# DearCaat/MHIM-MIL

Hardware: AMD Instinct MI355X
Metric: patch-instances/sec through MHIM fwd+bwd, N=10k D=1024 (higher is better)
Workload: dtype f32; 1 GPU; c2: MHIM(ABMIL) train step, one bag N=10000 D=1024 per GPU per step (teacher fwd + select + student fwd + bwd + Adam + EMA); rotating_bags_per_gpu=8, matrix_core_form=bf16x3, parallelism=dp1, launch=hipGraph replay, one graph per resident bag

## Files before the change

include/mhimx.h:

```cpp
#ifndef MHIMX_H
#define MHIMX_H

#include <stdint.h>

#ifdef __cplusplus
extern "C" {
#endif

#define MHIMX_VERSION 620

enum { MHIMX_ACT_NONE = 0, MHIMX_ACT_RELU = 1, MHIMX_ACT_GELU = 2, MHIMX_ACT_TANH = 3 };

enum { MHIMX_PREC_F32 = 0, MHIMX_PREC_F16S = 1, MHIMX_PREC_BF16X3 = 2 };

const char* mhimx_last_error(void);
int mhimx_version(void);


typedef struct {
  const float* A; int64_t lda; const int64_t* rows;
  const float* B; int64_t ldb;
  float* C; int64_t ldc;
  int64_t M, N, K;
  const float* bias;
// ... 282 lines not shown
                          float* colsum_out, int32_t accumulate, void* ws, int64_t ws_bytes, mhimx_reduce_list* defer );
int mhimx_rows_dpre_image_c(void* stream, const float* dH_compact, const void* dact16, const int64_t* rows, int64_t L, int64_t E, void* img,
                            float* colsum_out, int32_t accumulate, void* ws, int64_t ws_bytes, mhimx_reduce_list* defer );
int mhimx_rows_dpre_image_k(void* stream, const float* dH, const void* dact16, const uint8_t* keep, int64_t N, int64_t E, void* img,
                            float* colsum_out, int32_t accumulate, void* ws, int64_t ws_bytes, mhimx_reduce_list* defer );
typedef struct {
  const void* img;
  const float* X; int64_t ldx; int64_t n_bag_rows;
  const int64_t* rows;
  int64_t L, E, D;
  float* C; int64_t ldc; int32_t accumulate;
  float* ws; int64_t ws_floats;
  mhimx_reduce_list* defer;
  int32_t ride_tail;
  const void* ximg;
} mhimx_bag_wgrad_args;
int64_t mhimx_wgrad_ws_floats(int64_t L, int64_t E, int64_t D);
int mhimx_bag_wgrad(void* stream, const mhimx_bag_wgrad_args* a);
int64_t mhimx_wgrad_multi_ws_floats(int64_t L, int64_t E, int64_t D, int32_t n_bags);
int mhimx_bag_wgrad_multi(void* stream, const mhimx_bag_wgrad_args* bags, int32_t n_bags);
int mhimx_shard_flags(void* stream, const int64_t* rows_all, int64_t R, int64_t Lk, int64_t lo, int64_t n, int64_t k_tokens,
                      int32_t tokens_live, uint8_t* excl);
int mhimx_shard_gather(void* stream, const float* H, int64_t E, const int64_t* rows, int64_t R, int64_t lo, int64_t n, float* out);
int mhimx_shard_scatter(void* stream, const float* dX, int64_t E, const int64_t* rows, int64_t R, int64_t lo, int64_t n, float* dH);
int mhimx_colsum(void* stream, const float* X, int64_t M, int64_t E, float* out, int32_t accumulate,
                 void* ws, int64_t ws_bytes);

int mhimx_head_fwd_bwd(void* stream, const float* z, const float* t, const float* wp, const float* bp,
                       const int64_t* label_dev, int64_t E, int64_t C, float temp_t, float main_alpha,
                       float aux_alpha, float inv_accum, float* logits, float* losses, float* g_z, float* d_wp,
                       float* d_bp, int32_t accumulate, const float* g_logits_in, const float* g_cl_in);

int mhimx_softmax_cols(void* stream, const float* x, float* y, int64_t M, int64_t C, float alpha);
// ... 45 lines not shown
  int32_t act, da_act;
  int32_t attn2score;
  float drop_p_teacher, drop_p_student;
  float merge_drop_p, merge_mm;
  float temp_t, main_alpha, aux_alpha;
  mhimx_step_params student, teacher;
  mhimx_step_grads grad;
  float* p; float* g; float* m; float* v; float* p_teacher;
  int64_t n_train, n_all;
  float lr, beta1, beta2, eps, weight_decay, ema_mm;
  const float* mm_table; int64_t mm_len; const float* lr_table; int64_t lr_len;
  uint64_t* tick; uint64_t* opt_step;
  float* q_out;
  int32_t time_project;
  void* side_stream;
} mhimx_step_cfg;
typedef struct { int64_t k_top, n_sel, len_keep, Lk, R; } mhimx_step_counts;
int mhimx_step_counts_of(int64_t N, double mask_ratio_h, double mask_ratio_hr, double merge_ratio, mhimx_step_counts* out);
typedef struct { uint64_t drop_teacher, drop_student, select, mca; } mhimx_step_seeds;
typedef struct {
  int64_t total;
  int64_t logits, losses;
  int64_t score;
  int64_t rows_all;
  int64_t H_teacher, H_student;
  int64_t dact;
  int64_t z_teacher, z_student, g_z;
  int64_t dH;
} mhimx_step_layout;
int mhimx_step_layout_of(const mhimx_step_cfg* cfg, int64_t N, const mhimx_step_counts* cnt, mhimx_step_layout* out);
// ... 284 lines not shown
```

mhim_mil_amd/_lib.py:

```python
from __future__ import annotations

import ctypes as C
import os

HERE = os.path.dirname(os.path.abspath(__file__))
LIB_PATH = os.path.join(HERE, os.environ.get("MHIMX_LIB_NAME", "libmhimx.so"))

c_f32p = C.c_void_p
c_i64p = C.c_void_p
c_u8p = C.c_void_p

ABI_VERSION = 620

ACT = {None: 0, "none": 0, "identity": 0, "relu": 1, "gelu": 2, "tanh": 3}
PREC = {"f32": 0, "f16s": 1, "bf16x3": 2}


def act_code(name, allowed):
    n = name.lower() if isinstance(name, str) else None
    return ACT[n] if n in allowed else 0


class GemmNT(C.Structure):
    _fields_ = [("A", c_f32p), ("lda", C.c_int64), ("rows", c_i64p),
# ... 15 lines not shown


class ProjScore(C.Structure):
    _fields_ = [("wa16", c_f32p), ("wc", c_f32p), ("act", C.c_int32), ("C", C.c_int32), ("s", c_f32p), ("cproj", c_f32p),
                ("pm", c_f32p), ("pl", c_f32p), ("pz", c_f32p), ("xch", c_f32p), ("gate", C.c_void_p)]


class BagProject(C.Structure):
    _fields_ = [("X", c_f32p), ("ldx", C.c_int64), ("N", C.c_int64), ("D", C.c_int64), ("E", C.c_int64),
                ("act", C.c_int32), ("n_heads", C.c_int32), ("head", ProjHead * 2), ("drop_tick", C.c_void_p), ("score0", C.c_void_p)]


class BagWgrad(C.Structure):
    _fields_ = [("img", C.c_void_p), ("X", c_f32p), ("ldx", C.c_int64), ("n_bag_rows", C.c_int64), ("rows", C.c_void_p),
                ("L", C.c_int64), ("E", C.c_int64), ("D", C.c_int64), ("C", c_f32p), ("ldc", C.c_int64), ("accumulate", C.c_int32),
                ("ws", c_f32p), ("ws_floats", C.c_int64), ("defer", C.c_void_p), ("ride_tail", C.c_int32), ("ximg", C.c_void_p)]


class PpegBand(C.Structure):
    _fields_ = [("H", C.c_int64), ("cell0", C.c_int64), ("ncell", C.c_int64), ("out0", C.c_int64), ("out1", C.c_int64)]


class PrepJob(C.Structure):
    _fields_ = [("kind", C.c_int32), ("inp", C.c_void_p), ("out", C.c_void_p), ("R", C.c_int64), ("C", C.c_int64)]


class ReduceJob(C.Structure):
    _fields_ = [("kind", C.c_int32), ("accumulate", C.c_int32), ("parts", c_f32p), ("out", c_f32p),
                ("G", C.c_int64), ("W", C.c_int64), ("ld", C.c_int64), ("K1", C.c_int64), ("K2", C.c_int64), ("ldo", C.c_int64)]


# ... 100 lines not shown

class StepGrads(C.Structure):
    _fields_ = [(n, C.c_void_p) for n in ("w1", "b1", "wa", "wc", "wp", "bp", "ln_w", "ln_b", "wkv", "wq", "wo", "bo")]


class StepCfg(C.Structure):
    _fields_ = [("D", C.c_int64), ("E", C.c_int64), ("A", C.c_int64), ("C", C.c_int64), ("k", C.c_int64),
                ("act", C.c_int32), ("da_act", C.c_int32), ("attn2score", C.c_int32),
                ("drop_p_teacher", C.c_float), ("drop_p_student", C.c_float), ("merge_drop_p", C.c_float), ("merge_mm", C.c_float),
                ("temp_t", C.c_float), ("main_alpha", C.c_float), ("aux_alpha", C.c_float),
                ("student", StepParams), ("teacher", StepParams), ("grad", StepGrads),
                ("p", C.c_void_p), ("g", C.c_void_p), ("m", C.c_void_p), ("v", C.c_void_p), ("p_teacher", C.c_void_p),
                ("n_train", C.c_int64), ("n_all", C.c_int64),
                ("lr", C.c_float), ("beta1", C.c_float), ("beta2", C.c_float), ("eps", C.c_float), ("weight_decay", C.c_float), ("ema_mm", C.c_float),
                ("mm_table", C.c_void_p), ("mm_len", C.c_int64), ("lr_table", C.c_void_p), ("lr_len", C.c_int64),
                ("tick", C.c_void_p), ("opt_step", C.c_void_p), ("q_out", C.c_void_p), ("time_project", C.c_int32), ("side_stream", C.c_void_p)]


class StepCounts(C.Structure):
    _fields_ = [("k_top", C.c_int64), ("n_sel", C.c_int64), ("len_keep", C.c_int64), ("Lk", C.c_int64), ("R", C.c_int64)]


class StepSeeds(C.Structure):
    _fields_ = [("drop_teacher", C.c_uint64), ("drop_student", C.c_uint64), ("select", C.c_uint64), ("mca", C.c_uint64)]


class StepLayout(C.Structure):
    _fields_ = [(n, C.c_int64) for n in ("total", "logits", "losses", "score", "rows_all", "H_teacher", "H_student", "dact", "z_teacher",
                                        "z_student", "g_z", "dH")]


# ... 190 lines not shown
    "mhimx_dsmil_head": (C.c_int, [_P, _P, _P, _P, _P, _P, _I64, _I64, _F, _F, _F, _F, _P, _P, _P, _P, _P]),
    "mhimx_mul_colsum": (C.c_int, [_P, _P, _P, _I64, _I64, _P, _I32, _P, _I64, _P]),
    "mhimx_rows_dpre": (C.c_int, [_P, _P, _P, _P, _I64, _I64, _P, _P, _I32, _P, _I64, _P]),
    "mhimx_bmm_affine": (C.c_int, [_P, _I32, _P, _I32, _I64, _I64, _I64, C.c_float, C.c_float]),
    "mhimx_bmm_affine2": (C.c_int, [_P, _I32, _P, _I32, _I64, _I64, _I64, C.c_float, C.c_float, _P, C.c_float, C.c_float]),
    "mhimx_bmm_affine_pair": (C.c_int, [_P, _I32, C.POINTER(GemmNT), _F, _F, _I32, C.POINTER(GemmNT), _F, _F, _I32, _I64]),
    "mhimx_shard_flags": (C.c_int, [_P, _P, _I64, _I64, _I64, _I64, _I64, _I32, _P]),
    "mhimx_shard_gather": (C.c_int, [_P, _P, _I64, _P, _I64, _I64, _I64, _P]),
    "mhimx_shard_scatter": (C.c_int, [_P, _P, _I64, _P, _I64, _I64, _I64, _P]),
    "mhimx_rows_dpre_image": (C.c_int, [_P, _P, _P, _P, _I64, _I64, _P, _P, _I32, _P, _I64, _P]),
    "mhimx_rows_dpre_image_c": (C.c_int, [_P, _P, _P, _P, _I64, _I64, _P, _P, _I32, _P, _I64, _P]),
    "mhimx_rows_dpre_image_k": (C.c_int, [_P, _P, _P, _P, _I64, _I64, _P, _P, _I32, _P, _I64, _P]),
    "mhimx_wgrad_image_bytes": (_I64, [_I64, _I64]),
    "mhimx_wgrad_ws_floats": (_I64, [_I64, _I64, _I64]),
    "mhimx_bag_wgrad": (C.c_int, [_P, _P]),
    "mhimx_bag_wgrad_multi": (C.c_int, [_P, _P, _I32]),
    "mhimx_wgrad_multi_ws_floats": (C.c_int64, [_I64, _I64, _I64, _I32]),
    "mhimx_reduce_flush": (C.c_int, [_P, _P]),
    "mhimx_cls_metrics_ws_bytes": (C.c_int64, [_I64, _I64, _I64]),
    "mhimx_cls_metrics": (C.c_int, [_P, _P, _I64, _P, _I64, _I64, _I32, _P, _I64, _P, _P, _I64]),
    "mhimx_surv_nll": (C.c_int, [_P, _P, _I64, _P, _P, _I64, _I64, _F, _F, _F, _P, _P, _P]),
    "mhimx_cindex_ws_bytes": (C.c_int64, [_I64, _I64]),
    "mhimx_cindex": (C.c_int, [_P, _P, _P, _P, _I64, _P, _I64, _F, _P, _P, _I64]),
    "mhimx_colsum": (C.c_int, [_P, _P, _I64, _I64, _P, _I32, _P, _I64]),
    "mhimx_head_fwd_bwd": (C.c_int, [_P, _P, _P, _P, _P, _P, _I64, _I64, _F, _F, _F, _F, _P, _P, _P, _P, _P, _I32, _P, _P]),
    "mhimx_head_surv_fwd_bwd": (C.c_int, [_P, _P, _P, _P, _P, _P, _P, _I64, _I64, _F, _F, _F, _F, _F, _F, _P, _P, _P, _P, _P, _P, _I32]),
    "mhimx_adam_ema": (C.c_int, [_P, _P, _P, _P, _P, _P, _I64, _I64, _I64, _F, _F, _F, _F, _F, _F, _F, _I32, _P, _P, _I64]),
    "mhimx_bmm_chain": (C.c_int, [_P, C.POINTER(BmmStep), _I32, _I32, _P]),
    "mhimx_optim_step": (C.c_int, [_P, C.POINTER(OptimArgs)]),
    "mhimx_stream_copy": (C.c_int, [_P, _P, _P, _I64]),
# ... 110 lines not shown
```

mhim_mil_amd/csrc/step.hip:

```cpp
#include <math.h>
#include <string.h>

#include "infer_tab.hpp"
#include "step_mid.hpp"

namespace mhimx {

int64_t merge2_rows_tiles(int64_t R);

namespace {

struct DagEvents {
  hipEvent_t e[64][6];
  bool have[64] = {};
  int get(hipEvent_t** out) {
    int dev = 0;
    MHIMX_HIP(hipGetDevice(&dev));
    MHIMX_CHECK_ARG(dev >= 0 && dev < 64, "step: device index %d", dev);
    if (!have[dev]) {
      for (int i = 0; i < 6; ++i) MHIMX_HIP(hipEventCreateWithFlags(&e[dev][i], hipEventDisableTiming));
      have[dev] = true;
    }
    *out = e[dev];
    return 0;
// ... 389 lines not shown
  mhimx_reduce_list lst;
  memset(&lst, 0, sizeof(lst));
  const MidImg pimg = {cv.at<char>(b.img), dact, cv.at<float>(b.ws_b)};
  if (int r = mid_bwd_rows(stream, im, fwd, bag, c.grad, 0, fuse_img ? &pimg : nullptr, dag, &lst)) return r;
  mhimx_reduce_list lst_main;
  memset(&lst_main, 0, sizeof(lst_main));
  mhimx_reduce_list* lm = dag ? &lst_main : &lst;
  if (fuse_img) {
    if (int r = dpre_merge_rows(stream, dH, dact, rows_all, R, E, cv.at<char>(b.img), b.P0, c.grad.b1, cv.at<float>(b.ws_b), b.ws_b_bytes, lm)) return r;
  } else if (int r = mhimx_rows_dpre_image(stream, dH, dact, rows_all, len_keep, E, cv.at<char>(b.img), c.grad.b1, 0, cv.at<char>(b.ws_b), b.ws_b_bytes, lm))
    return r;
  {
    mhimx_bag_wgrad_args g = {};
    g.img = cv.at<char>(b.img); g.X = X; g.ldx = ldx; g.n_bag_rows = N; g.rows = fuse_img ? cv.at<int64_t>(b.rows_img) : rows_all; g.L = b.L_img; g.E = E; g.D = D;
    g.C = c.grad.w1; g.ldc = D;
    g.accumulate = 0; g.ws = cv.at<float>(b.wg_ws); g.ws_floats = b.wg_ws_floats; g.defer = lm; g.ride_tail = update ? 1 : 0;
    if (int r = mhimx_bag_wgrad(stream, &g)) return r;
  }
  if (dag)
    if (int r = dag_edge(dag->ev[4], dag->side_st, dag->main_st)) return r;
  if (!update) return mhimx_reduce_flush(stream, lm);

  mhimx_optim_args o = optim_args_of(c, host_step, true);
  o.fold = lm;
  return mhimx_optim_step(stream, &o);
}

namespace mhimx {
namespace {

struct QChainW { float wq; float w[MHIMX_WINDOW_MAX]; };
// ... 346 lines not shown

  mhimx_reduce_list lst;
  memset(&lst, 0, sizeof(lst));
  {
    mhimx_scorer sc_b = sc;
    sc_b.wa_frag = nullptr;
    mhimx_pool_grad pg = {};
    pg.g_z = g_z; pg.dT1 = dH; pg.d_wa = c.grad.wa; pg.d_wc = c.grad.wc; pg.wa_t = wa_t; pg.accumulate = 0; pg.splits = 8; pg.defer = &lst; pg.wa_t_frag = wa_t_frag;
    if (int r = mhimx_abmil_pool_bwd(stream, &sc_b, &io, &pg)) return r;
  }
  if (int r = mhimx_rows_dpre_image(stream, dH, dact, nullptr, N, E, cv.at<char>(b.img), c.grad.b1, 0, cv.at<char>(b.ws_b), b.ws_b_bytes, &lst)) return r;
  {
    mhimx_bag_wgrad_args g = {};
    g.img = cv.at<char>(b.img); g.X = X; g.ldx = ldx; g.n_bag_rows = N; g.rows = nullptr; g.L = N; g.E = E; g.D = D;
    g.C = c.grad.w1; g.ldc = D;
    g.accumulate = 0; g.ws = cv.at<float>(b.wg_ws); g.ws_floats = b.wg_ws_floats; g.defer = &lst; g.ride_tail = update ? 1 : 0;
    if (int r = mhimx_bag_wgrad(stream, &g)) return r;
  }
  if (!update) return mhimx_reduce_flush(stream, &lst);

  mhimx_optim_args o = optim_args_of(c, host_step, false);
  o.fold = &lst;
  return mhimx_optim_step(stream, &o);
}

extern "C" int mhimx_pure_step_run_many(void* stream, const mhimx_step_cfg* cfg, int32_t n_bags, const float* const* X, const int64_t* ldx, const int64_t* N,
                                        const int64_t* const* labels_dev, const uint64_t* drop_seeds, int64_t host_step0, void* ws, int64_t ws_bytes) {
  MHIMX_CHECK_ARG(n_bags >= 1 && X && ldx && N && labels_dev && drop_seeds, "pure_step_run_many: null arguments");
  for (int32_t i = 0; i < n_bags; ++i)
    if (int r = mhimx_pure_step_run(stream, cfg, X[i], ldx[i], N[i], labels_dev[i], drop_seeds[i], host_step0 + i, ws, ws_bytes, 1)) return r;
  return 0;
// ... 2 lines not shown
```

mhim_mil_amd/csrc/wgrad.hip:

```cpp
#include <string.h>

#include "mma_tile.hpp"
#include "mca2_side.hpp"
#include "reduce_jobs.hpp"

namespace mhimx {

constexpr int WBI = 128, WBN = 256, WBK = 32, WTHREADS = 512;
constexpr int WA_BYTES = WBI * 128, WB_BYTES = WBN * 128;
constexpr int W_MAX_CHUNK = 3072;
constexpr int WNF = 16;

#define WG_READ8(x, oa, ob, a, b)                                                                                       \
  asm volatile("ds_read_b128 %0, %8\n\tds_read_b128 %1, %8 offset:512\n\tds_read_b128 %2, %8 offset:1024\n\t"           \
               "ds_read_b128 %3, %8 offset:1536\n\t"                                                                    \
               "ds_read_b128 %4, %9\n\tds_read_b128 %5, %9 offset:1024\n\tds_read_b128 %6, %9 offset:2048\n\t"          \
               "ds_read_b128 %7, %9 offset:3072"                                                                        \
               : "=&v"(x[oa]), "=&v"(x[oa + 1]), "=&v"(x[oa + 2]), "=&v"(x[oa + 3]), "=&v"(x[ob]), "=&v"(x[ob + 1]),       \
                 "=&v"(x[ob + 2]), "=&v"(x[ob + 3])                                                                      \
               : "v"(a), "v"(b)                                                                                         \
               : "memory")
#define WG_WAIT8(n, x, oa, ob)                                                                                          \
  asm volatile("s_waitcnt lgkmcnt(" #n ")"                                                                              \
               : "+v"(x[oa]), "+v"(x[oa + 1]), "+v"(x[oa + 2]), "+v"(x[oa + 3]), "+v"(x[ob]), "+v"(x[ob + 1]),             \
// ... 292 lines not shown
        const int64_t n = n0 + 4 * (16 * (2 * wn + cb) + r16);
        *reinterpret_cast<f32x4*>(out + i * g.D + n) =
            f32x4{acc[ja][4 * cb + 0][e], acc[ja][4 * cb + 1][e], acc[ja][4 * cb + 2][e], acc[ja][4 * cb + 3][e]};
      }
#ifdef WG_PROF
  asm volatile("s_waitcnt vmcnt(0)" ::: "memory");
  if (bx == 0 && lane == 0) {
    const uint64_t wp_t3 = __builtin_readcyclecounter();
    float* pr = reinterpret_cast<float*>(const_cast<char*>(gimg) + (int64_t)g.ksteps * nIT * WA_BYTES) + wave * 4;
    pr[0] = (float)(wp_t1 - wp_t0); pr[1] = (float)(wp_t2 - wp_t1); pr[2] = (float)(wp_t3 - wp_t2); pr[3] = (float)nk;
    if (wave == 4) { pr[32 - 16] = (float)(wall_clock64() - wp_rt0); pr[33 - 16] = (float)(wp_t3 - wp_t0); }
  }
#endif
}

constexpr int DNS = 3, DSTAGE = WA_BYTES + WB_BYTES, DRING = DNS * DSTAGE;

__global__ __launch_bounds__(WTHREADS) void bag_wgrad_dma_kernel(WgradArgs g, const char* ximg, int side_blocks, Merge2Side side, WgradTail tail) {
  extern __shared__ __attribute__((aligned(16))) char smem[];
  if (wg_rider_block(smem, side_blocks, side, tail)) return;
  const unsigned bx = blockIdx.x - (unsigned)side_blocks;
  const int tid = threadIdx.x, lane = tid & 63, wave = tid >> 6;
  const int wm = wave >> 2, wn = wave & 3;
  const int nJ = (int)(g.D / WBN), nIT = (int)(g.E / WBI), nT = nIT * nJ;
  const int xcd = bx & 7, sidx = bx >> 3;
  const int slab = (sidx / nT) * 8 + xcd, tile = sidx % nT;
  if (slab >= g.splits) return;
  const int itile = tile / nJ, jtile = tile % nJ;
  const int64_t i0 = (int64_t)itile * WBI, n0 = (int64_t)jtile * WBN;
  const int ks0 = slab * g.kps;
// ... 108 lines not shown
      *reinterpret_cast<f32x4*>(tile + j * 512) = hi;
      *reinterpret_cast<f32x4*>(tile + j * 512 + 2048) = lo;
    }
  }
  if (part) {
    if (koct > 0) reinterpret_cast<f32x4*>(lds)[(koct - 1) * 64 + (tid & 63)] = cs;
    __syncthreads();
    if (koct == 0 && live) {
      const f32x4* o = reinterpret_cast<const f32x4*>(lds) + (tid & 63);
      cs = (cs + o[0]) + (o[64] + o[128]);
      reinterpret_cast<f32x4*>(part + (int64_t)ks * E)[cq] = cs;
    }
  }
}

static bool wgrad_shape_ok(int64_t L, int64_t E, int64_t D, int64_t ldx, int64_t n_bag_rows) {
  return L >= 1 && E >= WBI && E % WBI == 0 && D >= WBN && D % WBN == 0 && ldx % 4 == 0 && ldx >= D &&
         n_bag_rows * ldx * 4 < ((int64_t)1 << 32);
}

}

using namespace mhimx;

extern "C" int64_t mhimx_wgrad_image_bytes(int64_t L, int64_t E) { return cdiv(L, WBK) * WBK * E * 4; }

static int wgrad_plan(int64_t L, int64_t E, int64_t D, int* kps_out) {
  const int ksteps = (int)cdiv(L, WBK);
  const int64_t tiles = (E / WBI) * (D / WBN);
  int64_t want = cdiv(256, tiles);
  if (want > cdiv(ksteps, 4)) want = cdiv(ksteps, 4);
  if (want < 1) want = 1;
  int kps = (int)cdiv(ksteps, want);
  if (kps * WBK > W_MAX_CHUNK) kps = W_MAX_CHUNK / WBK;
  *kps_out = kps;
  return (int)cdiv(ksteps, kps);
}
extern "C" int64_t mhimx_wgrad_ws_floats(int64_t L, int64_t E, int64_t D) {
  int kps;
  return (int64_t)wgrad_plan(L, E, D, &kps) * E * D;
}

static int rows_dpre_image_impl(void* stream, const float* dH, const void* dact16, const int64_t* rows, int64_t L, int64_t E, void* img,
                                float* colsum_out, int32_t accumulate, void* ws, int64_t ws_bytes, mhimx_reduce_list* defer, int dh_compact,
// ... 38 lines not shown
  const int ksteps = (int)cdiv(L, WBK);
  const int64_t tiles = (E / WBI) * (D / WBN);
  int64_t spb = cdiv(256, tiles * n_bags);
  const int64_t need = cdiv((int64_t)ksteps * WBK, W_MAX_CHUNK);
  if (spb < need) spb = need;
  if (spb > ksteps) spb = ksteps;
  int kps = (int)cdiv(ksteps, spb);
  *kps_out = kps;
  return (int)cdiv(ksteps, kps);
}
extern "C" int64_t mhimx_wgrad_multi_ws_floats(int64_t L, int64_t E, int64_t D, int32_t n_bags) {
  int kps;
  return (int64_t)wgrad_plan_multi(L, E, D, n_bags, &kps) * n_bags * E * D;
}

static int bag_wgrad_impl(void* stream, const mhimx_bag_wgrad_args* bags, int n_bags) {
  const mhimx_bag_wgrad_args* a = bags;
  MHIMX_CHECK_ARG(a->img && a->X && a->C && a->ws && aligned16(a->img) && aligned16(a->X) && aligned16(a->C) && aligned16(a->ws) && a->ldc % 4 == 0,
                  "bag_wgrad: null / unaligned operand");
  MHIMX_CHECK_ARG(wgrad_shape_ok(a->L, a->E, a->D, a->ldx, a->n_bag_rows),
                  "bag_wgrad: needs E %% 128 == 0, D %% 256 == 0, 16-byte aligned rows and a bag below 4 GiB");
  WgradArgs g;
  g.img = (const char*)a->img; g.X = a->X; g.ldx = a->ldx; g.rows = a->rows; g.L = a->L; g.E = a->E; g.D = a->D;
  g.ksteps = (int)cdiv(a->L, WBK);
  WgradBags mb = {};
  if (n_bags == 1) {
    g.splits = wgrad_plan(a->L, a->E, a->D, &g.kps);
    mb.spb = g.splits;
  } else {
    mb.spb = wgrad_plan_multi(a->L, a->E, a->D, n_bags, &g.kps);
    g.splits = mb.spb * n_bags;
  }
  for (int b = 0; b < n_bags; ++b) {
    const mhimx_bag_wgrad_args& q = bags[b];
    MHIMX_CHECK_ARG(q.img && q.X && aligned16(q.img) && aligned16(q.X) && q.L == a->L && q.E == a->E && q.D == a->D && q.ldx == a->ldx &&
                        q.n_bag_rows * q.ldx * 4 < ((int64_t)1 << 32) && (q.rows != nullptr) == (a->rows != nullptr),
                    "bag_wgrad_multi: bag %d: null / unaligned operand, or not the shape of bag 0 (L, E, D, ldx, row ids)", b);
    mb.img[b] = (const char*)q.img; mb.X[b] = q.X; mb.rows[b] = q.rows;
  }
  MHIMX_CHECK_ARG(a->ws_floats >= (int64_t)g.splits * a->E * a->D, "bag_wgrad: workspace too small (%lld floats)", (long long)((int64_t)g.splits * a->E * a->D));
  g.out = a->ws;
  const size_t smem = SRING + (size_t)g.kps * WBK * 4;
  Merge2Side side = {};
  int side_blocks = 0;
  mhimx_reduce_list* defer = a->defer;
  if (defer && defer->side.pending == 2 && smem >= M2_SIDE_LDS * sizeof(float)) {
    memcpy(&side, defer->side.blob, sizeof(side));
    side_blocks = merge2_side_blocks(2, side);
    if (side_blocks % 8 == 0) defer->side.pending = 3;
    else side_blocks = 0;
  }
  const int64_t tiles = (a->E / WBI) * (a->D / WBN);
  dim3 grid((unsigned)(8 * tiles * cdiv(g.splits, 8) + side_blocks));
  WgradTail tail = {};
  MHIMX_CHECK_ARG(!a->ximg || (n_bags == 1 && !a->rows && aligned16(a->ximg) && a->L == a->n_bag_rows),
                  "bag_wgrad: the bag image (ximg) goes with a bag-ordered dPRE image: one bag, no row list, L = n_bag_rows");
  if (a->ride_tail && defer && n_bags == 1 && (defer->n > 0 || defer->side.pending == 3)) {
    for (int i = 0; i < defer->n; ++i) {
      const mhimx_reduce_job& j = defer->j[i];
      MHIMX_CHECK_ARG(j.parts && j.out && j.G > 0 && (j.kind == 0 ? j.W > 0 : (j.kind == 1 && j.K1 > 0 && j.K2 > 0)), "bag_wgrad: bad queued reduction %d", i);
    }
    tail.first = (int)grid.x;
    tail.n_reduce = reduce_table_fill(tail.t, defer->j, defer->n, WTHREADS);
    defer->n = 0;
    if (defer->side.pending == 3 && side_blocks > 0) {
      tail.stage3 = merge2_side_blocks(3, side);
      tail.gate_want = side_blocks;
      defer->side.pending = 0;
    }
    grid.x += (unsigned)(tail.n_reduce + tail.stage3);
  }
  if (a->ximg) {
    MHIMX_ONCE_PER_DEVICE(MHIMX_HIP(hipFuncSetAttribute((const void*)bag_wgrad_dma_kernel, hipFuncAttributeMaxDynamicSharedMemorySize, DRING)));
    hipLaunchKernelGGL(bag_wgrad_dma_kernel, grid, dim3(WTHREADS), DRING, (hipStream_t)stream, g, (const char*)a->ximg, side_blocks, side, tail);
  } else {
    MHIMX_ONCE_PER_DEVICE(MHIMX_HIP(hipFuncSetAttribute((const void*)bag_wgrad_ws_kernel, hipFuncAttributeMaxDynamicSharedMemorySize, SRING + W_MAX_CHUNK * 4)));
    hipLaunchKernelGGL(bag_wgrad_ws_kernel, grid, dim3(WTHREADS), smem, (hipStream_t)stream, g, mb, side_blocks, side, tail);
  }
  MHIMX_LAUNCH_CHECK();
  if (!defer_push(defer, reduce_job_slabs(a->ws, g.splits, a->E, a->D, a->ldc, a->C, a->accumulate))) {
    const int rc = reduce_slabs_now((hipStream_t)stream, a->ws, a->C, a->E, a->D, a->ldc, g.splits, a->accumulate);
    if (rc) return rc;
  }
  return 0;
}

extern "C" int mhimx_bag_wgrad(void* stream, const mhimx_bag_wgrad_args* a) {
  if (!a) return fail(-1, "bag_wgrad: null argument block");
  return bag_wgrad_impl(stream, a, 1);
// ... 6 lines not shown
```

mhim_mil_amd/engine.py:

```python
from __future__ import annotations

from typing import Optional

import collections
import contextlib
import dataclasses
import os

import torch

from . import mhim as mh
from . import ops
from .mhim import MHIM, BagPlan


class CommonMIL:

    def __init__(self, args=None, fused=None, graph_cache=0) -> None:
        self.training = True
        self.fused = fused
        self.graph_cache = int(graph_cache)

    def _native_step(self, tr, bag, label, n_iter, extra):
        if self.graph_cache > 0 and not extra:
# ... 401 lines not shown
            self._split = 0
        student._tick = self.tick
        if teacher is not None:
            teacher._tick = self.tick
        self.mm_table = None if mm_sche is None else torch.as_tensor(mm_sche, dtype=torch.float32).to(dev).contiguous()
        self.clip_grad = None if clip_grad is None else float(clip_grad)
        self.lr_table = None if lr_sche is None else torch.as_tensor(lr_sche, dtype=torch.float32).to(dev).contiguous()
        self._clip_ws = torch.empty(1024, device=dev) if self.clip_grad else None
        self._g_extra = None
        self._fold_now, self._fold_list = False, None
        self._graph_pool = None
        self._cap_stream = None
        self._side = None
        self.step_dag = os.environ.get("MHIMX_STEP_DAG", "0") != "0"
        self.use_executor = os.environ.get("MHIMX_STEP_EXEC", "1") != "0"
        self._exec, self.time_project = None, False
        self.exec_max_rows = 262144
        self.single_pass = True
        self.window_streams = 4
        self.window_batched = _WINDOW_BATCHED
        self._win, self._win_w, self._shape_graphs = None, {}, None
        self._rows_cache = {}
        self.pure_window_row_cap = 262144
        self.ragged_window_row_cap = 262144
        self.dsmil_window_row_cap = 131072
        self._dsmil_exec = None
        self.dsmil_mhim_window_row_cap = 131072
        self._dsmil_mhim_exec = None

    def _dist(self):
# ... 470 lines not shown
        if not mhim:
            return ex
        if self.step_dag:
            if self._side is None or self._side.device != fl.student.device:
                self._side = torch.cuda.Stream(device=fl.student.device)
            cfg.side_stream = self._side.cuda_stream
        else:
            cfg.side_stream = None
        if self._chain is not None:
            if self._q_scratch is None:
                self._q_scratch = torch.empty((s.merge.k, s.mlp_dim), device=fl.student.device)
            cfg.q_out = self._q_scratch.data_ptr()
        else:
            cfg.q_out = None
        cfg.time_project = int(bool(self.time_project))
        cfg.attn2score = int(bool(t.attn2score))
        cfg.drop_p_teacher = float(t.dropout_p if t.training else 0.0)
        cfg.merge_drop_p, cfg.merge_mm = float(s.merge.dropout), float(s.merge.g_q_mm)
        cfg.temp_t, cfg.aux_alpha = float(s.temp_t), float(self.aux_alpha)
        cfg.p_teacher = None if fl.same_teacher else fl.teacher.data_ptr()
        cfg.mm_table, cfg.mm_len = (None, 0) if self.mm_table is None else (self.mm_table.data_ptr(), self.mm_table.numel())
        return ex

    def _exec_window_ok(self, xs, labels, i=None):
        n = len(xs)
        if not (self.window_batched and 2 <= n <= _L.WINDOW_MAX and self.world == 1 and self._chain is None and not self.step_dag
                and self.flat.n_all % 4 == 0 and self.s.merge.k <= 6 and self.s.mrh_sche is None and self.flat.names[0] == "feature.0.weight"):
            return False
        x0 = xs[0]
        if not (x0.dim() == 2 and x0.shape[0] <= 16384 and all(x.shape == x0.shape and x.stride() == x0.stride() and x.device == x0.device for x in xs)):
# ... 660 lines not shown
```

mhim_mil_amd/ops.py:

```python
from __future__ import annotations

import collections
import ctypes as C
import functools
import itertools
import math
from typing import Optional

import torch

from . import _lib as L


KERNEL_EVENT_HOOK = None


import threading

_PIN = threading.local()


def _pinned():
    st = getattr(_PIN, "stream", None)
    if st is not None and getattr(_PIN, "device", -1) == torch.cuda.current_device():
# ... 598 lines not shown

def bag_wgrad_ok(x, E, n_rows):
    return (n_rows >= 1 and E % 128 == 0 and x.shape[1] % 256 == 0 and x.stride(0) % 4 == 0
            and x.shape[0] * x.stride(0) * 4 < (1 << 32))


def bag_ximage_floats(x):
    return -(-x.shape[0] // 32) * 32 * x.shape[1]


def bag_wgrad_ximg_ok(x, E):
    return x.dim() == 2 and x.is_contiguous() and x.shape[1] % 256 == 0 and E % 128 == 0


def bag_wgrad(dH, dact16, x, rows, n_rows, out_w=None, out_b=None, accumulate=False, defer=None, rows_dh="same", want_bias=True,
              dh_compact=False, ride_tail=False, ximg=None, keep=None):
    _chk(dH, name="dH"); _chk(dact16, torch.float16, "dact16"); _chk(rows, torch.int64, "rows")
    if not (x.is_cuda and x.dtype == torch.float32 and x.dim() == 2 and x.stride(1) == 1):
        raise L.MhimxError("x: expected a GPU fp32 matrix with contiguous rows")
    if ximg is not None:
        _chk(ximg, name="ximg"); _chk(keep, torch.uint8, "keep")
        N, E, D = x.shape[0], dH.shape[1], x.shape[1]
        if not bag_wgrad_ximg_ok(x, E) or ximg.numel() < bag_ximage_floats(x) or (keep is not None and keep.numel() < N):
            raise L.MhimxError("bag_wgrad(ximg=): contiguous bag, D % 256 == 0, E % 128 == 0, image / keep flags of the bag's size")
        dev, lib = dH.device, L.lib()
        if out_w is None:
            out_w = torch.empty((E, D), device=dev)
        if out_b is None and want_bias:
            out_b = torch.empty(E, device=dev)
        img = torch.empty(lib.mhimx_wgrad_image_bytes(N, E) // 4, device=dev)
        ws_b = torch.empty(-(-N // 32) * E, device=dev) if want_bias else None
        L.check(lib.mhimx_rows_dpre_image_k(_stream(), _p(dH), _p(dact16), _p(keep), N, E, _p(img), _p(out_b) if want_bias else None,
                                            int(bool(accumulate)), _p(ws_b), ws_b.numel() * 4 if want_bias else 0, _dp(defer)), "mhimx_rows_dpre_image_k")
        ws = torch.empty(lib.mhimx_wgrad_ws_floats(N, E, D), device=dev)
        g = L.BagWgrad(img=_p(img), X=_p(x), ldx=x.stride(0), n_bag_rows=N, rows=None, L=N, E=E, D=D, C=_p(out_w), ldc=out_w.stride(0),
                       accumulate=int(bool(accumulate)), ws=_p(ws), ws_floats=ws.numel(), defer=_dp(defer),
                       ride_tail=int(bool(ride_tail and defer is not None)), ximg=_p(ximg))
        L.check(lib.mhimx_bag_wgrad(_stream(), C.byref(g)), "mhimx_bag_wgrad")
        if defer is not None:
            defer.keep.extend((ws_b, ws, img))
        return out_w, out_b
    rows_h = rows if isinstance(rows_dh, str) else rows_dh
    _chk(rows_h, torch.int64, "rows_dh")
    E, D = dH.shape[1], x.shape[1]
    n_rows = int(n_rows)
    dev = dH.device
    lib = L.lib()
    if out_w is None:
        out_w = torch.empty((E, D), device=dev)
    if out_b is None and want_bias:
        out_b = torch.empty(E, device=dev)
    img = torch.empty(lib.mhimx_wgrad_image_bytes(n_rows, E) // 4, device=dev)
    ws_b = torch.empty(-(-n_rows // 32) * E, device=dev) if want_bias else None
    fn = lib.mhimx_rows_dpre_image_c if dh_compact else lib.mhimx_rows_dpre_image
    L.check(fn(_stream(), _p(dH), _p(dact16), _p(rows_h), n_rows, E, _p(img), _p(out_b) if want_bias else None,
                                      int(bool(accumulate)), _p(ws_b), ws_b.numel() * 4 if want_bias else 0, _dp(defer)), "mhimx_rows_dpre_image")
    ws = torch.empty(lib.mhimx_wgrad_ws_floats(n_rows, E, D), device=dev)
    g = L.BagWgrad(img=_p(img), X=_p(x), ldx=x.stride(0), n_bag_rows=x.shape[0], rows=_p(rows), L=n_rows, E=E, D=D, C=_p(out_w),
                   ldc=out_w.stride(0), accumulate=int(bool(accumulate)), ws=_p(ws), ws_floats=ws.numel(), defer=_dp(defer),
                   ride_tail=int(bool(ride_tail and defer is not None)))
    L.check(lib.mhimx_bag_wgrad(_stream(), C.byref(g)), "mhimx_bag_wgrad")
    if defer is not None:
        defer.keep.extend((ws_b, ws, img))
    return out_w, out_b


class WgradImage:

    def __init__(self, img, x, rows, n_rows, E, keep):
        self.img, self.x, self.rows, self.n_rows, self.E, self.keep = img, x, rows, int(n_rows), int(E), keep


def bag_wgrad_image(dH, dact16, x, rows, n_rows, out_b=None, accumulate=False, defer=None):
    _chk(dH, name="dH"); _chk(dact16, torch.float16, "dact16"); _chk(rows, torch.int64, "rows")
    E = dH.shape[1]
# ... 688 lines not shown
```

Before: 32.46 million patch-instances/s.

## Add two-workgroups-per-CU weight-gradient kernel with narrower tiles and smaller LDS ring

Adds a bag_wgrad_ws2_kernel variant using 128-column B tiles and a 2-deep A/B LDS ring sized so two workgroups fit per CU. Producer waves stream X rows through registers with a three-register-set rotation, and consumer waves run bf16x3 MFMA. An automatic form selector picks it for single bags when the tile × split count stays within twice the CU count; a new form field lets callers force either kernel. The aim is better latency hiding and occupancy for the X^T·dpre weight-gradient GEMM, at the cost of shallower buffering and more tiles per split.

```diff
diff --git a/include/mhimx.h b/include/mhimx.h
--- a/include/mhimx.h
+++ b/include/mhimx.h
@@ -320,9 +320,11 @@
   mhimx_reduce_list* defer;
   int32_t ride_tail;
   const void* ximg;
+  int32_t form;
 } mhimx_bag_wgrad_args;
 int64_t mhimx_wgrad_ws_floats(int64_t L, int64_t E, int64_t D);
 int mhimx_bag_wgrad(void* stream, const mhimx_bag_wgrad_args* a);
+int32_t mhimx_bag_wgrad_form(const mhimx_bag_wgrad_args* a, int32_t n_bags);
 int64_t mhimx_wgrad_multi_ws_floats(int64_t L, int64_t E, int64_t D, int32_t n_bags);
 int mhimx_bag_wgrad_multi(void* stream, const mhimx_bag_wgrad_args* bags, int32_t n_bags);
 int mhimx_shard_flags(void* stream, const int64_t* rows_all, int64_t R, int64_t Lk, int64_t lo, int64_t n, int64_t k_tokens,
@@ -398,6 +400,7 @@
   float* q_out;
   int32_t time_project;
   void* side_stream;
+  int32_t wgrad_form;
 } mhimx_step_cfg;
 typedef struct { int64_t k_top, n_sel, len_keep, Lk, R; } mhimx_step_counts;
 int mhimx_step_counts_of(int64_t N, double mask_ratio_h, double mask_ratio_hr, double merge_ratio, mhimx_step_counts* out);
diff --git a/mhim_mil_amd/_lib.py b/mhim_mil_amd/_lib.py
--- a/mhim_mil_amd/_lib.py
+++ b/mhim_mil_amd/_lib.py
@@ -53,7 +53,7 @@
 class BagWgrad(C.Structure):
     _fields_ = [("img", C.c_void_p), ("X", c_f32p), ("ldx", C.c_int64), ("n_bag_rows", C.c_int64), ("rows", C.c_void_p),
                 ("L", C.c_int64), ("E", C.c_int64), ("D", C.c_int64), ("C", c_f32p), ("ldc", C.c_int64), ("accumulate", C.c_int32),
-                ("ws", c_f32p), ("ws_floats", C.c_int64), ("defer", C.c_void_p), ("ride_tail", C.c_int32), ("ximg", C.c_void_p)]
+                ("ws", c_f32p), ("ws_floats", C.c_int64), ("defer", C.c_void_p), ("ride_tail", C.c_int32), ("ximg", C.c_void_p), ("form", C.c_int32)]
 
 
 class PpegBand(C.Structure):
@@ -184,7 +184,7 @@
                 ("n_train", C.c_int64), ("n_all", C.c_int64),
                 ("lr", C.c_float), ("beta1", C.c_float), ("beta2", C.c_float), ("eps", C.c_float), ("weight_decay", C.c_float), ("ema_mm", C.c_float),
                 ("mm_table", C.c_void_p), ("mm_len", C.c_int64), ("lr_table", C.c_void_p), ("lr_len", C.c_int64),
-                ("tick", C.c_void_p), ("opt_step", C.c_void_p), ("q_out", C.c_void_p), ("time_project", C.c_int32), ("side_stream", C.c_void_p)]
+                ("tick", C.c_void_p), ("opt_step", C.c_void_p), ("q_out", C.c_void_p), ("time_project", C.c_int32), ("side_stream", C.c_void_p), ("wgrad_form", C.c_int32)]
 
 
 class StepCounts(C.Structure):
@@ -405,6 +405,7 @@
     "mhimx_wgrad_image_bytes": (_I64, [_I64, _I64]),
     "mhimx_wgrad_ws_floats": (_I64, [_I64, _I64, _I64]),
     "mhimx_bag_wgrad": (C.c_int, [_P, _P]),
+    "mhimx_bag_wgrad_form": (_I32, [_P, _I32]),
     "mhimx_bag_wgrad_multi": (C.c_int, [_P, _P, _I32]),
     "mhimx_wgrad_multi_ws_floats": (C.c_int64, [_I64, _I64, _I64, _I32]),
     "mhimx_reduce_flush": (C.c_int, [_P, _P]),
diff --git a/mhim_mil_amd/csrc/step.hip b/mhim_mil_amd/csrc/step.hip
--- a/mhim_mil_amd/csrc/step.hip
+++ b/mhim_mil_amd/csrc/step.hip
@@ -427,7 +427,7 @@
     mhimx_bag_wgrad_args g = {};
     g.img = cv.at<char>(b.img); g.X = X; g.ldx = ldx; g.n_bag_rows = N; g.rows = fuse_img ? cv.at<int64_t>(b.rows_img) : rows_all; g.L = b.L_img; g.E = E; g.D = D;
     g.C = c.grad.w1; g.ldc = D;
-    g.accumulate = 0; g.ws = cv.at<float>(b.wg_ws); g.ws_floats = b.wg_ws_floats; g.defer = lm; g.ride_tail = update ? 1 : 0;
+    g.accumulate = 0; g.ws = cv.at<float>(b.wg_ws); g.ws_floats = b.wg_ws_floats; g.defer = lm; g.ride_tail = update ? 1 : 0; g.form = c.wgrad_form;
     if (int r = mhimx_bag_wgrad(stream, &g)) return r;
   }
   if (dag)
@@ -804,7 +804,7 @@
     mhimx_bag_wgrad_args g = {};
     g.img = cv.at<char>(b.img); g.X = X; g.ldx = ldx; g.n_bag_rows = N; g.rows = nullptr; g.L = N; g.E = E; g.D = D;
     g.C = c.grad.w1; g.ldc = D;
-    g.accumulate = 0; g.ws = cv.at<float>(b.wg_ws); g.ws_floats = b.wg_ws_floats; g.defer = &lst; g.ride_tail = update ? 1 : 0;
+    g.accumulate = 0; g.ws = cv.at<float>(b.wg_ws); g.ws_floats = b.wg_ws_floats; g.defer = &lst; g.ride_tail = update ? 1 : 0; g.form = c.wgrad_form;
     if (int r = mhimx_bag_wgrad(stream, &g)) return r;
   }
   if (!update) return mhimx_reduce_flush(stream, &lst);
diff --git a/mhim_mil_amd/csrc/wgrad.hip b/mhim_mil_amd/csrc/wgrad.hip
--- a/mhim_mil_amd/csrc/wgrad.hip
+++ b/mhim_mil_amd/csrc/wgrad.hip
@@ -330,6 +330,196 @@
 #endif
 }
 
+constexpr int W2BN = 128, W2B_BYTES = W2BN * 128;
+constexpr int S2NA = 2, S2NB = 2, S2RING = S2NA * WA_BYTES + S2NB * W2B_BYTES;
+constexpr int W2_MAX_LDS = 81920;
+static_assert(S2RING + W_MAX_CHUNK * 4 <= W2_MAX_LDS, "ring + the largest row table must leave room for a second workgroup");
+static_assert(M2_SIDE_LDS * 4 <= S2RING && 32 * 33 * 4 <= S2RING, "the riders' LDS must fit the smaller launch");
+
+MHIMX_DEV void ws2_unit(const f32x4 (&a)[4], const f32x4 (&b)[4], f32x4 (&acc)[4][4]) {
+#pragma unroll
+  for (int i = 0; i < 4; ++i)
+#pragma unroll
+    for (int j = 0; j < 4; ++j) acc[i][j] = mt_mfma(a[i], b[j], acc[i][j]);
+}
+
+__global__ __launch_bounds__(WTHREADS, 2) void bag_wgrad_ws2_kernel(WgradArgs g, int side_blocks, Merge2Side side, WgradTail tail) {
+  extern __shared__ __attribute__((aligned(16))) char smem[];
+  if (wg_rider_block(smem, side_blocks, side, tail)) return;
+  const unsigned bx = blockIdx.x - (unsigned)side_blocks;
+  const int tid = threadIdx.x, lane = tid & 63, wave = tid >> 6;
+#ifdef WG_PROF
+  const uint64_t wp_t0 = __builtin_readcyclecounter();
+  const uint64_t wp_rt0 = wall_clock64();
+#endif
+  const int nJ = (int)(g.D / W2BN), nIT = (int)(g.E / WBI), nT = nIT * nJ;
+  const int xcd = bx & 7, sidx = bx >> 3;
+  const int slab = (sidx / nT) * 8 + xcd, tile = sidx % nT;
+  if (slab >= g.splits) return;
+  const int itile = tile / nJ;
+  const int64_t i0 = (int64_t)itile * WBI, n0 = (int64_t)(tile % nJ) * W2BN;
+  const int ks0 = slab * g.kps;
+  const int nk = (ks0 + g.kps < g.ksteps ? ks0 + g.kps : g.ksteps) - ks0;
+  unsigned* rowtab = reinterpret_cast<unsigned*>(smem + S2RING);
+  for (int q = tid; q < nk * WBK; q += WTHREADS) {
+    int64_t l = (int64_t)ks0 * WBK + q;
+    if (l >= g.L) l = g.L - 1;
+    rowtab[q] = (unsigned)((g.rows ? g.rows[l] : l) * g.ldx * 4);
+  }
+  __syncthreads();
+  const unsigned lds0 = (unsigned)(uintptr_t)(lptr_f)smem;
+
+  if (wave < 4) {
+    const int oct = wave, half = lane >> 5, c = lane & 31;
+    const unsigned colb = (unsigned)((n0 + 4 * c) * 4);
+    typedef unsigned u32x4 __attribute__((ext_vector_type(4)));
+    struct XSet { f32x4 v[4]; };
+    const float* const gX = g.X;
+    const char* const gA = g.img + ((int64_t)ks0 * nIT + itile) * WA_BYTES;
+    const unsigned astep = (unsigned)(nIT * WA_BYTES), apiece = (unsigned)((wave * 64 + lane) * 16);
+    auto row_offsets = [&](int t) {
+      return *reinterpret_cast<const u32x4*>(reinterpret_cast<const char*>(rowtab) + (oct * 8 + half * 4) * 4 + (t < nk ? t : nk - 1) * 128);
+    };
+    auto load_x_async = [&](int t, XSet& r) {
+      const u32x4 ro = row_offsets(t);
+      asm volatile("global_load_dwordx4 %0, %4, %8\n\tglobal_load_dwordx4 %1, %5, %8\n\tglobal_load_dwordx4 %2, %6, %8\n\t"
+                   "global_load_dwordx4 %3, %7, %8"
+                   : "=&v"(r.v[0]), "=&v"(r.v[1]), "=&v"(r.v[2]), "=&v"(r.v[3])
+                   : "v"(ro[0] + colb), "v"(ro[1] + colb), "v"(ro[2] + colb), "v"(ro[3] + colb), "s"(gX)
+                   : "memory");
+    };
+    const unsigned xs0 = (unsigned)(S2NA * WA_BYTES + ((oct * 2) * 128 + (2 * half) * 32 + c) * 16);
+    auto store_x = [&](int t, XSet& r) {
+      char* sb = smem + (t % S2NB) * W2B_BYTES + xs0;
+      float a[4][4];
+#pragma unroll
+      for (int q = 0; q < 4; ++q) {
+        a[q][0] = r.v[q][0]; a[q][1] = r.v[q][1]; a[q][2] = r.v[q][2]; a[q][3] = r.v[q][3];
+        wg_swap(a[q][0], a[q][2]);
+        wg_swap(a[q][1], a[q][3]);
+      }
+#pragma unroll
+      for (int sx = 0; sx < 2; ++sx) {
+        const float kv[8] = {a[0][sx], a[1][sx], a[2][sx], a[3][sx], a[0][sx + 2], a[1][sx + 2], a[2][sx + 2], a[3][sx + 2]};
+        f32x4 hi, lo;
+        wg_split8(kv, hi, lo);
+        *reinterpret_cast<f32x4*>(sb + sx * 512) = hi;
+        *reinterpret_cast<f32x4*>(sb + sx * 512 + 2048) = lo;
+      }
+    };
+    auto issue_a = [&](int t, bool live) {
+      char* sa = smem + (t % S2NA) * WA_BYTES + wave * 1024;
+      const char* src = live ? gA + (int64_t)t * astep + apiece : g.img;
+#pragma unroll
+      for (int j = 0; j < 4; ++j)
+        __builtin_amdgcn_global_load_lds((gptr_f)(live ? src + j * 4096 : src), (lptr_f)(sa + j * 4096), 16, 0, 0);
+    };
+    XSet s0, s1, s2;
+    issue_a(0, true);
+    {
+      const char* xb = reinterpret_cast<const char*>(gX);
+      const u32x4 ro = row_offsets(0);
+      XSet r0;
+#pragma unroll
+      for (int q = 0; q < 4; ++q) r0.v[q] = *reinterpret_cast<const f32x4*>(xb + ro[q] + colb);
+      store_x(0, r0);
+    }
+    load_x_async(1, s1);
+    issue_a(1, false);
+    load_x_async(2, s2);
+    asm volatile("s_waitcnt vmcnt(12) lgkmcnt(0)" ::: "memory");
+    __builtin_amdgcn_s_barrier();
+#define WS2_SET(s) "+v"(s.v[0]), "+v"(s.v[1]), "+v"(s.v[2]), "+v"(s.v[3])
+    auto body = [&](int t, XSet& r_load, XSet& r_use) {
+      issue_a(t + 1, t + 1 < nk);
+      load_x_async(t + 3, r_load);
+      asm volatile("s_waitcnt vmcnt(16)" : WS2_SET(r_use) : : "memory");
+      if (t + 1 < nk) store_x(t + 1, r_use);
+      asm volatile("s_waitcnt vmcnt(4) lgkmcnt(0)" ::: "memory");
+      __builtin_amdgcn_s_barrier();
+    };
+#ifdef WG_PROF
+    const uint64_t wp_t1 = __builtin_readcyclecounter();
+#endif
+    int t = 0;
+#pragma unroll 1
+    for (; t + 2 < nk; t += 3) {
+      body(t, s0, s1);
+      body(t + 1, s1, s2);
+      body(t + 2, s2, s0);
+    }
+    if (t < nk) body(t, s0, s1);
+    if (t + 1 < nk) body(t + 1, s1, s2);
+    asm volatile("s_waitcnt vmcnt(0)" : WS2_SET(s0), WS2_SET(s1), WS2_SET(s2) : : "memory");
+#undef WS2_SET
+#ifdef WG_PROF
+    if (bx == 0 && lane == 0) {
+      const uint64_t wp_t2 = __builtin_readcyclecounter();
+      float* pr = reinterpret_cast<float*>(const_cast<char*>(g.img) + (int64_t)g.ksteps * nIT * WA_BYTES) + wave * 4;
+      pr[0] = (float)(wp_t1 - wp_t0); pr[1] = (float)(wp_t2 - wp_t1); pr[2] = 0.f; pr[3] = (float)nk;
+    }
+#endif
+    return;
+  }
+
+  const int cw = wave - 4, wm = cw >> 1, wn = cw & 1;
+  const int r16 = lane & 15, kg = lane >> 4;
+  const unsigned fa_hi = lds0 + ((kg * 2) * 128 + 16 * wm + r16) * 16, fa_lo = fa_hi + 2048;
+  const unsigned fb_hi = lds0 + S2NA * WA_BYTES + ((kg * 2) * 128 + 16 * wn + r16) * 16, fb_lo = fb_hi + 2048;
+  f32x4 acc[4][4];
+#pragma unroll
+  for (int i = 0; i < 4; ++i)
+#pragma unroll
+    for (int j = 0; j < 4; ++j) acc[i][j] = f32x4{0.f, 0.f, 0.f, 0.f};
+  f32x4 P[4], Q[4], R[4];
+  __builtin_amdgcn_s_barrier();
+#ifdef WG_PROF
+  const uint64_t wp_t1 = __builtin_readcyclecounter();
+#endif
+#pragma unroll 1
+  for (int t = 0; t < nk; ++t) {
+    const unsigned ca = (unsigned)((t % S2NA) * WA_BYTES), cb = (unsigned)((t % S2NB) * W2B_BYTES);
+    WS_READ4A(P, fa_lo + ca);
+    WS_READ4A(Q, fb_hi + cb);
+    WS_READ4A(R, fa_hi + ca);
+    WS_WAIT8(4, P, Q);
+    __builtin_amdgcn_sched_barrier(0);
+    ws2_unit(P, Q, acc);
+    __builtin_amdgcn_sched_barrier(0);
+    WS_READ4A(P, fb_lo + cb);
+    WS_WAIT8(4, R, Q);
+    __builtin_amdgcn_sched_barrier(0);
+    ws2_unit(R, Q, acc);
+    __builtin_amdgcn_sched_barrier(0);
+    WS_WAIT8(0, R, P);
+    __builtin_amdgcn_sched_barrier(0);
+    ws2_unit(R, P, acc);
+    __builtin_amdgcn_sched_barrier(0);
+    __builtin_amdgcn_s_barrier();
+  }
+#ifdef WG_PROF
+  const uint64_t wp_t2 = __builtin_readcyclecounter();
+#endif
+  float* out = g.out + (int64_t)slab * g.E * g.D;
+#pragma unroll
+  for (int ja = 0; ja < 4; ++ja)
+#pragma unroll
+    for (int e = 0; e < 4; ++e) {
+      const int64_t i = i0 + 4 * (16 * wm + 4 * kg + e) + ja;
+      const int64_t n = n0 + 4 * (16 * wn + r16);
+      *reinterpret_cast<f32x4*>(out + i * g.D + n) = f32x4{acc[ja][0][e], acc[ja][1][e], acc[ja][2][e], acc[ja][3][e]};
+    }
+#ifdef WG_PROF
+  asm volatile("s_waitcnt vmcnt(0)" ::: "memory");
+  if (bx == 0 && lane == 0) {
+    const uint64_t wp_t3 = __builtin_readcyclecounter();
+    float* pr = reinterpret_cast<float*>(const_cast<char*>(g.img) + (int64_t)g.ksteps * nIT * WA_BYTES) + wave * 4;
+    pr[0] = (float)(wp_t1 - wp_t0); pr[1] = (float)(wp_t2 - wp_t1); pr[2] = (float)(wp_t3 - wp_t2); pr[3] = (float)nk;
+    if (wave == 4) { pr[32 - 16] = (float)(wall_clock64() - wp_rt0); pr[33 - 16] = (float)(wp_t3 - wp_t0); }
+  }
+#endif
+}
+
 constexpr int DNS = 3, DSTAGE = WA_BYTES + WB_BYTES, DRING = DNS * DSTAGE;
 
 __global__ __launch_bounds__(WTHREADS) void bag_wgrad_dma_kernel(WgradArgs g, const char* ximg, int side_blocks, Merge2Side side, WgradTail tail) {
@@ -468,8 +658,8 @@
   }
 }
 
-static bool wgrad_shape_ok(int64_t L, int64_t E, int64_t D, int64_t ldx, int64_t n_bag_rows) {
-  return L >= 1 && E >= WBI && E % WBI == 0 && D >= WBN && D % WBN == 0 && ldx % 4 == 0 && ldx >= D &&
+static bool wgrad_shape_ok(int64_t L, int64_t E, int64_t D, int64_t ldx, int64_t n_bag_rows, int bn = WBN) {
+  return L >= 1 && E >= WBI && E % WBI == 0 && D >= bn && D % bn == 0 && ldx % 4 == 0 && ldx >= D &&
          n_bag_rows * ldx * 4 < ((int64_t)1 << 32);
 }
 
@@ -481,7 +671,7 @@
 
 static int wgrad_plan(int64_t L, int64_t E, int64_t D, int* kps_out) {
   const int ksteps = (int)cdiv(L, WBK);
-  const int64_t tiles = (E / WBI) * (D / WBN);
+  const int64_t tiles = (E / WBI) * cdiv(D, WBN);
   int64_t want = cdiv(256, tiles);
   if (want > cdiv(ksteps, 4)) want = cdiv(ksteps, 4);
   if (want < 1) want = 1;
@@ -550,11 +740,26 @@
   return (int64_t)wgrad_plan_multi(L, E, D, n_bags, &kps) * n_bags * E * D;
 }
 
+static bool wgrad_two_per_cu(const mhimx_bag_wgrad_args* a, int n_bags) {
+  if (a->form == 1 || n_bags != 1 || a->ximg || !wgrad_shape_ok(a->L, a->E, a->D, a->ldx, a->n_bag_rows, W2BN)) return false;
+  if (a->form == 2 || !wgrad_shape_ok(a->L, a->E, a->D, a->ldx, a->n_bag_rows)) return true;
+  int kps;
+  return (a->E / WBI) * (a->D / W2BN) * wgrad_plan(a->L, a->E, a->D, &kps) <= 2 * 256;
+}
+extern "C" int32_t mhimx_bag_wgrad_form(const mhimx_bag_wgrad_args* a, int32_t n_bags) {
+  if (!a || n_bags < 1 || n_bags > W_MAX_BAGS || a->form < 0 || a->form > 2) return -1;
+  if (wgrad_two_per_cu(a, n_bags)) return 2;
+  return a->form != 2 && wgrad_shape_ok(a->L, a->E, a->D, a->ldx, a->n_bag_rows) ? 1 : -1;
+}
+
 static int bag_wgrad_impl(void* stream, const mhimx_bag_wgrad_args* bags, int n_bags) {
   const mhimx_bag_wgrad_args* a = bags;
   MHIMX_CHECK_ARG(a->img && a->X && a->C && a->ws && aligned16(a->img) && aligned16(a->X) && aligned16(a->C) && aligned16(a->ws) && a->ldc % 4 == 0,
                   "bag_wgrad: null / unaligned operand");
-  MHIMX_CHECK_ARG(wgrad_shape_ok(a->L, a->E, a->D, a->ldx, a->n_bag_rows),
+  MHIMX_CHECK_ARG(a->form >= 0 && a->form <= 2, "bag_wgrad: form is 0 (automatic), 1 (one workgroup per CU) or 2 (two per CU)");
+  const bool two = wgrad_two_per_cu(a, n_bags);
+  MHIMX_CHECK_ARG(a->form != 2 || two, "bag_wgrad: form 2 takes one bag without ximg, E %% 128 == 0, D %% 128 == 0, 16-byte aligned rows, a bag below 4 GiB");
+  MHIMX_CHECK_ARG(two || wgrad_shape_ok(a->L, a->E, a->D, a->ldx, a->n_bag_rows),
                   "bag_wgrad: needs E %% 128 == 0, D %% 256 == 0, 16-byte aligned rows and a bag below 4 GiB");
   WgradArgs g;
   g.img = (const char*)a->img; g.X = a->X; g.ldx = a->ldx; g.rows = a->rows; g.L = a->L; g.E = a->E; g.D = a->D;
@@ -576,7 +781,7 @@
   }
   MHIMX_CHECK_ARG(a->ws_floats >= (int64_t)g.splits * a->E * a->D, "bag_wgrad: workspace too small (%lld floats)", (long long)((int64_t)g.splits * a->E * a->D));
   g.out = a->ws;
-  const size_t smem = SRING + (size_t)g.kps * WBK * 4;
+  const size_t smem = (two ? S2RING : SRING) + (size_t)g.kps * WBK * 4;
   Merge2Side side = {};
   int side_blocks = 0;
   mhimx_reduce_list* defer = a->defer;
@@ -586,7 +791,7 @@
     if (side_blocks % 8 == 0) defer->side.pending = 3;
     else side_blocks = 0;
   }
-  const int64_t tiles = (a->E / WBI) * (a->D / WBN);
+  const int64_t tiles = (a->E / WBI) * (a->D / (two ? W2BN : WBN));
   dim3 grid((unsigned)(8 * tiles * cdiv(g.splits, 8) + side_blocks));
   WgradTail tail = {};
   MHIMX_CHECK_ARG(!a->ximg || (n_bags == 1 && !a->rows && aligned16(a->ximg) && a->L == a->n_bag_rows),
@@ -609,6 +814,9 @@
   if (a->ximg) {
     MHIMX_ONCE_PER_DEVICE(MHIMX_HIP(hipFuncSetAttribute((const void*)bag_wgrad_dma_kernel, hipFuncAttributeMaxDynamicSharedMemorySize, DRING)));
     hipLaunchKernelGGL(bag_wgrad_dma_kernel, grid, dim3(WTHREADS), DRING, (hipStream_t)stream, g, (const char*)a->ximg, side_blocks, side, tail);
+  } else if (two) {
+    MHIMX_ONCE_PER_DEVICE(MHIMX_HIP(hipFuncSetAttribute((const void*)bag_wgrad_ws2_kernel, hipFuncAttributeMaxDynamicSharedMemorySize, W2_MAX_LDS)));
+    hipLaunchKernelGGL(bag_wgrad_ws2_kernel, grid, dim3(WTHREADS), smem, (hipStream_t)stream, g, side_blocks, side, tail);
   } else {
     MHIMX_ONCE_PER_DEVICE(MHIMX_HIP(hipFuncSetAttribute((const void*)bag_wgrad_ws_kernel, hipFuncAttributeMaxDynamicSharedMemorySize, SRING + W_MAX_CHUNK * 4)));
     hipLaunchKernelGGL(bag_wgrad_ws_kernel, grid, dim3(WTHREADS), smem, (hipStream_t)stream, g, mb, side_blocks, side, tail);
diff --git a/mhim_mil_amd/engine.py b/mhim_mil_amd/engine.py
--- a/mhim_mil_amd/engine.py
+++ b/mhim_mil_amd/engine.py
@@ -439,6 +439,7 @@
         self._side = None
         self.step_dag = os.environ.get("MHIMX_STEP_DAG", "0") != "0"
         self.use_executor = os.environ.get("MHIMX_STEP_EXEC", "1") != "0"
+        self.wgrad_form = 0
         self._exec, self.time_project = None, False
         self.exec_max_rows = 262144
         self.single_pass = True
@@ -939,6 +940,7 @@
         else:
             cfg.q_out = None
         cfg.time_project = int(bool(self.time_project))
+        cfg.wgrad_form = int(self.wgrad_form)
         cfg.attn2score = int(bool(t.attn2score))
         cfg.drop_p_teacher = float(t.dropout_p if t.training else 0.0)
         cfg.merge_drop_p, cfg.merge_mm = float(s.merge.dropout), float(s.merge.g_q_mm)
diff --git a/mhim_mil_amd/ops.py b/mhim_mil_amd/ops.py
--- a/mhim_mil_amd/ops.py
+++ b/mhim_mil_amd/ops.py
@@ -636,7 +636,7 @@
 
 
 def bag_wgrad(dH, dact16, x, rows, n_rows, out_w=None, out_b=None, accumulate=False, defer=None, rows_dh="same", want_bias=True,
-              dh_compact=False, ride_tail=False, ximg=None, keep=None):
+              dh_compact=False, ride_tail=False, ximg=None, keep=None, form=0):
     _chk(dH, name="dH"); _chk(dact16, torch.float16, "dact16"); _chk(rows, torch.int64, "rows")
     if not (x.is_cuda and x.dtype == torch.float32 and x.dim() == 2 and x.stride(1) == 1):
         raise L.MhimxError("x: expected a GPU fp32 matrix with contiguous rows")
@@ -657,7 +657,7 @@
         ws = torch.empty(lib.mhimx_wgrad_ws_floats(N, E, D), device=dev)
         g = L.BagWgrad(img=_p(img), X=_p(x), ldx=x.stride(0), n_bag_rows=N, rows=None, L=N, E=E, D=D, C=_p(out_w), ldc=out_w.stride(0),
                        accumulate=int(bool(accumulate)), ws=_p(ws), ws_floats=ws.numel(), defer=_dp(defer),
-                       ride_tail=int(bool(ride_tail and defer is not None)), ximg=_p(ximg))
+                       ride_tail=int(bool(ride_tail and defer is not None)), ximg=_p(ximg), form=int(form))
         L.check(lib.mhimx_bag_wgrad(_stream(), C.byref(g)), "mhimx_bag_wgrad")
         if defer is not None:
             defer.keep.extend((ws_b, ws, img))
@@ -680,7 +680,7 @@
     ws = torch.empty(lib.mhimx_wgrad_ws_floats(n_rows, E, D), device=dev)
     g = L.BagWgrad(img=_p(img), X=_p(x), ldx=x.stride(0), n_bag_rows=x.shape[0], rows=_p(rows), L=n_rows, E=E, D=D, C=_p(out_w),
                    ldc=out_w.stride(0), accumulate=int(bool(accumulate)), ws=_p(ws), ws_floats=ws.numel(), defer=_dp(defer),
-                   ride_tail=int(bool(ride_tail and defer is not None)))
+                   ride_tail=int(bool(ride_tail and defer is not None)), form=int(form))
     L.check(lib.mhimx_bag_wgrad(_stream(), C.byref(g)), "mhimx_bag_wgrad")
     if defer is not None:
         defer.keep.extend((ws_b, ws, img))
```

New measurement: 33.07 million patch-instances/s (median of 6 runs). 1.02x the previous value.
